# toonsegers/verifiable_mpc

Hardware: AMD Instinct MI355X
Metric: Ed25519 MSM scalar-mults/sec (higher is better)
Workload: dtype u32 (255-bit modular integers as 10 limbs of 25.5 bits, 32x32->64 multiply-adds)

## Files before the change

verifiable_mpc_amd/csrc/api.hip:

```cpp
#include <stdlib.h>

#include "common.h"


thread_local char vmpc_err_buf[512] = {0};

__attribute__((constructor)) static void vmpc_hw_queues_default() { setenv("GPU_MAX_HW_QUEUES", "16", 0); }

int vmpc_fr_check_dev(vmpc_ctx *ctx, const void *v, size_t n);

extern "C" const char *vmpc_last_error(void) { return vmpc_err_buf; }

const char *vmpc_getenv_experimental(const char *name) {
    const char *on = getenv("VMPC_EXPERIMENTAL");
    return (on && atoi(on) != 0) ? getenv(name) : nullptr;
}

extern "C" int vmpc_backend_info(char *buf, size_t buflen) {
    int n = 0;
    hipError_t e = hipGetDeviceCount(&n);
    if (e != hipSuccess || n <= 0) {
        if (buf && buflen) snprintf(buf, buflen, "no HIP device (%s)", hipGetErrorString(e));
        return VMPC_E_NODEV;
    }
    if (buf && buflen) {
        hipDeviceProp_t p;
        if (hipGetDeviceProperties(&p, 0) == hipSuccess)
            snprintf(buf, buflen, "%s %s cus=%d lds=%zu hbm=%.0fGiB devices=%d", p.gcnArchName, p.name,
                     p.multiProcessorCount, (size_t)p.sharedMemPerBlock,
                     (double)p.totalGlobalMem / (1024.0 * 1024.0 * 1024.0), n);
        else
            snprintf(buf, buflen, "devices=%d", n);
    }
    return n;
}

extern "C" int vmpc_ctx_create(int device, vmpc_ctx **out) {
    if (!out) return VMPC_E_INVAL;
    int n = 0;
    if (hipGetDeviceCount(&n) != hipSuccess || n <= 0) {
        snprintf(vmpc_err_buf, sizeof vmpc_err_buf, "no HIP device visible");
        return VMPC_E_NODEV;
    }
    if (device < 0 || device >= n) return VMPC_E_INVAL;
    VMPC_HIP_CHECK(hipSetDevice(device));
    vmpc_ctx *c = new vmpc_ctx();
    c->device = device;
    hipDeviceProp_t p;
    if (hipGetDeviceProperties(&p, device) == hipSuccess) {
        c->cu_count = p.multiProcessorCount;
        c->lds_optin = p.sharedMemPerBlockOptin ? p.sharedMemPerBlockOptin : p.sharedMemPerBlock;
    }
    hipError_t e = hipStreamCreateWithFlags(&c->stream, hipStreamNonBlocking);
    if (e != hipSuccess) {
        delete c;
        snprintf(vmpc_err_buf, sizeof vmpc_err_buf, "hipStreamCreate: %s", hipGetErrorString(e));
        return VMPC_E_HIP;
    }
    c->own_stream = true;
    e = hipMalloc((void **)&c->d_status, (VMPC_ST_WORDS + 16) * sizeof(uint32_t));
    if (e == hipSuccess) e = hipMemset(c->d_status, 0, (VMPC_ST_WORDS + 16) * sizeof(uint32_t));
    if (e != hipSuccess) {
        VMPC_IGNORE(hipStreamDestroy(c->stream));
        delete c;
        snprintf(vmpc_err_buf, sizeof vmpc_err_buf, "hipMalloc(status): %s", hipGetErrorString(e));
        return VMPC_E_HIP;
    }
    const char *w = getenv("VMPC_MSM_WINDOW");
    if (w) c->window_override = atoi(w);
    const char *fj = getenv("VMPC_FOLD_JUMP_DIGITS");
    if (fj && atoi(fj) == 4) c->fold_jump_digit_bits = 4;
    const char *sp = getenv("VMPC_SHORT_PATH");
    if (sp) c->short_path = atoi(sp) != 0;
    const char *bw = vmpc_getenv_experimental("VMPC_BUCKET_WGS_PER_CU");
    if (bw && atoi(bw) >= 0) c->bucket_wgs_per_cu = atoi(bw);
    const char *sf = vmpc_getenv_experimental("VMPC_SORT_FINE_BITS");
    if (sf && atoi(sf) >= 0) c->sort_fine_bits = atoi(sf);
    const char *rc = vmpc_getenv_experimental("VMPC_REDUCE_MAX_CHUNKS");
    if (rc && atoi(rc) >= 256 && atoi(rc) <= 32768) c->reduce_max_chunks = atoi(rc);
    const char *ro = vmpc_getenv_experimental("VMPC_REDUCE_CHUNKS");
    if (ro && atoi(ro) >= 64 && atoi(ro) <= 32768 && (atoi(ro) & (atoi(ro) - 1)) == 0) c->reduce_chunks_override = atoi(ro);
    const char *rt = vmpc_getenv_experimental("VMPC_REDUCE_TREE");
    if (rt) c->reduce_tree = atoi(rt) != 0;
    const char *ss = vmpc_getenv_experimental("VMPC_SEG_SHIFT_MIN");
    if (ss && atoi(ss) <= 0 && atoi(ss) >= -5) c->seg_shift_min = atoi(ss);
    *out = c;
    return VMPC_OK;
}

extern "C" int vmpc_ctx_destroy(vmpc_ctx *ctx) {
    if (!ctx) return VMPC_E_INVAL;
    if (ctx->p4_pool_busy) {
        snprintf(vmpc_err_buf, sizeof vmpc_err_buf, "vmpc_ctx_destroy: a vmpc_p4 of this context is still alive");
        return VMPC_E_INVAL;
    }
    VMPC_IGNORE(hipSetDevice(ctx->device));
    VMPC_IGNORE(hipStreamSynchronize(ctx->stream));
    for (auto &s : ctx->stages)
        for (auto &pr : s.pending) {
            VMPC_IGNORE(hipEventDestroy(pr.first));
            VMPC_IGNORE(hipEventDestroy(pr.second));
        }
    for (auto e : ctx->event_pool) VMPC_IGNORE(hipEventDestroy(e));
    if (ctx->xevent) VMPC_IGNORE(hipEventDestroy(ctx->xevent));
    if (ctx->ev_sorted) VMPC_IGNORE(hipEventDestroy(ctx->ev_sorted));
    if (ctx->ev_bucketed) VMPC_IGNORE(hipEventDestroy(ctx->ev_bucketed));
    if (ctx->pin_event) VMPC_IGNORE(hipEventDestroy(ctx->pin_event));
    if (ctx->pin) VMPC_IGNORE(hipHostFree(ctx->pin));
    if (ctx->ws) VMPC_IGNORE(hipFree(ctx->ws));
    if (ctx->p4_pool) VMPC_IGNORE(hipFree(ctx->p4_pool));
    if (ctx->p4_kblock) VMPC_IGNORE(hipFree(ctx->p4_kblock));
    if (ctx->d_status) VMPC_IGNORE(hipFree(ctx->d_status));
    if (ctx->short_cursors) VMPC_IGNORE(hipFree(ctx->short_cursors));
    if (ctx->ntt_twiddles) VMPC_IGNORE(hipFree(ctx->ntt_twiddles));
    if (ctx->own_stream) VMPC_IGNORE(hipStreamDestroy(ctx->stream));
    delete ctx;
    return VMPC_OK;
}

extern "C" int vmpc_ctx_set_stream(vmpc_ctx *ctx, void *hip_stream) {
    if (!ctx) return VMPC_E_INVAL;
    VMPC_HIP_CHECK(hipSetDevice(ctx->device));
    VMPC_HIP_CHECK(hipStreamSynchronize(ctx->stream));
    if (ctx->own_stream) {
        VMPC_IGNORE(hipStreamDestroy(ctx->stream));
        ctx->own_stream = false;
    }
    if (hip_stream) {
        ctx->stream = (hipStream_t)hip_stream;
    } else {
        VMPC_HIP_CHECK(hipStreamCreateWithFlags(&ctx->stream, hipStreamNonBlocking));
        ctx->own_stream = true;
    }
    return VMPC_OK;
}

extern "C" int vmpc_ctx_sync(vmpc_ctx *ctx) {
    if (!ctx) return VMPC_E_INVAL;
    VMPC_HIP_CHECK(hipSetDevice(ctx->device));
    VMPC_CHECK(vmpc_pinned_reserve(ctx, 0));
    volatile uint32_t *st = (volatile uint32_t *)((char *)ctx->pin_out + 2048);
    VMPC_HIP_CHECK(hipMemcpyAsync((void *)st, ctx->d_status, VMPC_ST_WORDS * sizeof(uint32_t), hipMemcpyDeviceToHost,
                                  ctx->stream));
    VMPC_HIP_CHECK(hipStreamSynchronize(ctx->stream));
    if (st[VMPC_ST_NONCANON]) {
        snprintf(vmpc_err_buf, sizeof vmpc_err_buf, "%u non-canonical scalar(s) (>= l) seen on device",
                 (unsigned)st[VMPC_ST_NONCANON]);
        VMPC_HIP_CHECK(hipMemsetAsync(ctx->d_status, 0, VMPC_ST_WORDS * sizeof(uint32_t), ctx->stream));
        VMPC_HIP_CHECK(hipStreamSynchronize(ctx->stream));
        return VMPC_E_NONCANON;
    }
    if (st[VMPC_ST_SHORT_OVERFLOW]) {
        snprintf(vmpc_err_buf, sizeof vmpc_err_buf,
                 "the short-commitment path met scalars beyond its fixed capacities: repeat the call on the general path "
                 "(vmpc_ctx_set_short_path(ctx, 0))");
        VMPC_HIP_CHECK(hipMemsetAsync(ctx->d_status, 0, VMPC_ST_WORDS * sizeof(uint32_t), ctx->stream));
        VMPC_HIP_CHECK(hipStreamSynchronize(ctx->stream));
        ctx->short_backoff = 64;
        return VMPC_E_AGAIN;
    }
    return VMPC_OK;
}

extern "C" int vmpc_ctx_debug_hold_wait(vmpc_ctx *ctx, int on) {
    if (!ctx) return VMPC_E_INVAL;
    ctx->stream_waits = on != 0;
    return VMPC_OK;
}

#define VMPC_DEBUG_DELAY_MAX_US 20000u
#define VMPC_DEBUG_DELAY_POLLS_PER_US 4u
__global__ __launch_bounds__(64) void k_debug_delay(uint32_t ticks, uint32_t max_polls) {
    if (threadIdx.x != 0) return;
    const uint64_t t0 = __builtin_amdgcn_s_memrealtime();
    for (uint32_t i = 0; i < max_polls; i++) {
        if (__builtin_amdgcn_s_memrealtime() - t0 >= (uint64_t)ticks) break;
        __builtin_amdgcn_s_sleep(16);
    }
}

extern "C" int vmpc_stream_debug_delay(void *hip_stream, int device, unsigned microseconds) {
    if (!hip_stream) return VMPC_E_INVAL;
    if (microseconds > VMPC_DEBUG_DELAY_MAX_US) {
        snprintf(vmpc_err_buf, sizeof vmpc_err_buf, "debug delay of %u us: the cap is %u us", microseconds,
                 VMPC_DEBUG_DELAY_MAX_US);
        return VMPC_E_RANGE;
    }
    if (microseconds == 0) return VMPC_OK;
    VMPC_HIP_CHECK(hipSetDevice(device));
    k_debug_delay<<<1, 64, 0, (hipStream_t)hip_stream>>>(microseconds * 100u,
                                                          microseconds * VMPC_DEBUG_DELAY_POLLS_PER_US + 64u);
    VMPC_KERNEL_CHECK();
    return VMPC_OK;
}

extern "C" int vmpc_ctx_debug_delay(vmpc_ctx *ctx, unsigned microseconds) {
    if (!ctx) return VMPC_E_INVAL;
    if (microseconds == 0 || microseconds > VMPC_DEBUG_DELAY_MAX_US)
        return vmpc_stream_debug_delay((void *)ctx->stream, ctx->device, microseconds);
    vmpc_stage_scope s(ctx, "debug_delay");
    return vmpc_stream_debug_delay((void *)ctx->stream, ctx->device, microseconds);
}

extern "C" int vmpc_ctx_set_short_path(vmpc_ctx *ctx, int on) {
    if (!ctx) return VMPC_E_INVAL;
    ctx->short_path = on ? 1 : 0;
    if (on == 2) ctx->short_backoff = 0;
    return VMPC_OK;
}

extern "C" int vmpc_ctx_get_short_path(vmpc_ctx *ctx, int *on) {
    if (!ctx || !on) return VMPC_E_INVAL;
    *on = ctx->short_path;
    return VMPC_OK;
}

extern "C" int vmpc_ctx_query(vmpc_ctx *ctx, int *done) {
    if (!ctx || !done) return VMPC_E_INVAL;
    VMPC_HIP_CHECK(hipSetDevice(ctx->device));
    hipError_t e = hipStreamQuery(ctx->stream);
    if (e == hipSuccess) {
        *done = 1;
    } else if (e == hipErrorNotReady) {
        (void)hipGetLastError();
        *done = 0;
    } else {
        VMPC_HIP_CHECK(e);
    }
    return VMPC_OK;
}

extern "C" int vmpc_ctx_wait_for(vmpc_ctx *waiter, vmpc_ctx *other) {
    if (!waiter || !other) return VMPC_E_INVAL;
    if (waiter == other || waiter->stream == other->stream) return VMPC_OK;
    VMPC_HIP_CHECK(hipSetDevice(other->device));
    if (!other->xevent) VMPC_HIP_CHECK(hipEventCreateWithFlags(&other->xevent, hipEventDisableTiming));
// ... 347 lines not shown
```

verifiable_mpc_amd/csrc/common.h:

```cpp
#pragma once
#include <hip/hip_runtime.h>
#include <stdint.h>
#include <stdio.h>
#include <string.h>

#include <string>
#include <vector>

#include "../../include/vmpc.h"

extern thread_local char vmpc_err_buf[512];

#define VMPC_HIP_CHECK(expr)                                                                  \
    do {                                                                                      \
        hipError_t _e = (expr);                                                               \
        if (_e != hipSuccess) {                                                               \
            snprintf(vmpc_err_buf, sizeof vmpc_err_buf, "%s:%d: %s -> %s", __FILE__, __LINE__, \
                     #expr, hipGetErrorString(_e));                                           \
            return VMPC_E_HIP;                                                                \
        }                                                                                     \
    } while (0)

#define VMPC_CHECK(expr)              \
    do {                              \
        int _r = (expr);              \
        if (_r != VMPC_OK) return _r; \
    } while (0)

#define VMPC_ST_NONCANON 0
#define VMPC_ST_SHORT_OVERFLOW 1
#define VMPC_ST_WORDS 4

struct vmpc_stage {
    const char *name;
    double ms = 0;
    uint64_t launches = 0;
    std::vector<std::pair<hipEvent_t, hipEvent_t>> pending;
};

struct vmpc_ctx {
    int device = 0;
    hipStream_t stream = nullptr;
    bool own_stream = false;
    void *ws = nullptr;
    size_t ws_bytes = 0;
    size_t ws_used = 0;
    uint32_t *d_status = nullptr;
    int window_override = 0;
    int bucket_wgs_per_cu = 0;
    int reduce_max_chunks = 32768;
    int reduce_chunks_override = 0;
    int short_path = 1;
    int short_backoff = 0;
    size_t lds_optin = 0;
    int fold_jump_digit_bits = 8;
    bool sort_wide_ready = false;
    bool short_ready = false;
    uint32_t *short_cursors = nullptr;
    int reduce_tree = 1;
    bool reduce_tree_ready = false;
    int seg_shift_min = -3;
    int sort_fine_bits = -1;
    int plan_fill_shift = 0;
    int cu_count = 256;
    vmpc_sort_view sort_view = {};
    bool sort_view_valid = false;
    hipEvent_t xevent = nullptr;
    hipStream_t bucket_stream = nullptr;
    hipEvent_t ev_sorted = nullptr, ev_bucketed = nullptr;
    hipStream_t stage_stream = nullptr;
    void *pin = nullptr;
    size_t pin_bytes = 0;
    hipEvent_t pin_event = nullptr;
    bool stream_waits = false;
    uint32_t *done_flag_dev = nullptr;
    uint32_t done_seq = 0;
    uint32_t p4_seq = 0;
    void *pin_out = nullptr;
    void *pin_out_dev = nullptr;
    void *p4_pool = nullptr;
    size_t p4_pool_bytes = 0;
    bool p4_pool_busy = false;
    void *p4_kblock = nullptr;
    int p4_kblock_rows = 0;
    uint8_t p4_kblock_key[64] = {0};
    int poly_product = 0;
    void *ntt_twiddles = nullptr;
    size_t ntt_arena_cap = 0;
    bool profile = false;
    std::vector<vmpc_stage> stages;
    std::vector<hipEvent_t> event_pool;
};

int vmpc_ws_reserve(vmpc_ctx *ctx, size_t total_bytes);
inline void *vmpc_ws_take(vmpc_ctx *ctx, size_t bytes) {
    size_t off = (ctx->ws_used + 255) & ~(size_t)255;
    ctx->ws_used = off + bytes;
    return (char *)ctx->ws + off;
}
int vmpc_stage_h2d(vmpc_ctx *ctx, void *dst, const void *src, size_t bytes);
int vmpc_pinned_reserve(vmpc_ctx *ctx, size_t bytes);
inline size_t vmpc_align(size_t b) { return (b + 255) & ~(size_t)255; }

int vmpc_ntt_poly_mul(vmpc_ctx *ctx, const void *a, size_t a_stride, size_t na, const void *b, size_t b_stride,
                      size_t nb, size_t k_lo, size_t k_cnt, void *out, size_t out_stride, size_t n_wit);

int vmpc_stage_begin(vmpc_ctx *ctx, const char *name);
void vmpc_stage_end(vmpc_ctx *ctx, int handle);

struct vmpc_stage_scope {
    vmpc_ctx *ctx;
    int h;
    vmpc_stage_scope(vmpc_ctx *c, const char *name) : ctx(c), h(vmpc_stage_begin(c, name)) {}
    ~vmpc_stage_scope() { vmpc_stage_end(ctx, h); }
};

const char *vmpc_getenv_experimental(const char *name);

#define VMPC_IGNORE(expr) ((void)(expr))
#define VMPC_KERNEL_CHECK() VMPC_HIP_CHECK(hipGetLastError())

#ifdef __HIPCC__
__device__ __forceinline__ void vmpc_publish_done(uint32_t *counter, uint32_t *flag, uint32_t seq) {
    __threadfence_system();
    if (atomicAdd(counter, 1u) == gridDim.x - 1) {
        *counter = 0;
        __threadfence_system();
        *(volatile uint32_t *)flag = seq;
    }
}
#endif
```

verifiable_mpc_amd/csrc/msm_reduce_tree.hip:

```cpp
#include "common.h"
#include "msm_sort.h"
#include "ge25519.h"
#include "ptio.h"
#include "quad.h"

#include "rt_tree.h"

template <bool HAS_U, bool LANE_P1>
__global__ void __launch_bounds__(LANE_P1 ? RT_THREADS / 2 : RT_THREADS)
k_msm_reduce_tree(const uint32_t *__restrict__ buckets, const uint32_t *__restrict__ counts, int nb, int G, int L,
                  uint32_t *__restrict__ out3) {
    extern __shared__ __align__(16) uint32_t rt_lds[];
    uint32_t *TA = rt_lds;
    uint32_t *RR = TA + RT_LEAVES * EXT_WORDS;
    uint32_t *DD = RR + (RT_LEAVES / 2) * EXT_WORDS;
    uint32_t *US = DD + (RT_LEAVES / 2) * EXT_WORDS;
    const int w = blockIdx.y, g = blockIdx.x;
    if (LANE_P1) {
        if (threadIdx.x < RT_LEAVES) {
            const int t = threadIdx.x;
            const int lo = (RT_LEAVES * g + t) * L;
            const uint32_t *bw = buckets + EXT_WORDS * ((size_t)w * nb + lo);
            const uint32_t *cw = counts + (size_t)w * (nb + 1) + lo + 1;
            ge_ext acc = ge_ext_identity(), sum = ge_ext_identity();
            bool have = false;
            for (int j = L - 1; j >= 0; j--) {
                if (cw[j]) {
                    const ge_ext B = ext_ld(bw + EXT_WORDS * j);
                    acc = have ? ge_add(acc, B) : B;
                    have = true;
                }
                if (j == L - 1) sum = acc;
                else if (have) sum = ge_add(sum, acc);
            }
            ext_st(TA + EXT_WORDS * t, acc);
            if (HAS_U) ext_st(US + EXT_WORDS * t, sum);
        }
    } else {
        const int t = threadIdx.x >> 2, q = threadIdx.x & 3;
        const int lo = (RT_LEAVES * g + t) * L;
        const uint32_t *bw = buckets + EXT_WORDS * ((size_t)w * nb + lo);
        const uint32_t *cw = counts + (size_t)w * (nb + 1) + lo + 1;
        fe acc = rt_identity(q), sum = acc;
        bool have = false;
        for (int j = L - 1; j >= 0; j--) {
            if (cw[j]) {
                const fe B = fe_ld(bw + EXT_WORDS * j + FE_LIMBS * q);
                acc = have ? rt_add(acc, B, q) : B;
                have = true;
            }
            if (HAS_U) {
                if (j == L - 1) sum = acc;
                else if (have) sum = rt_add(sum, acc, q);
            }
        }
        rt_st(TA, t, q, acc);
        if (HAS_U) rt_st(US, t, q, sum);
    }
    __syncthreads();
    rt_tree<!HAS_U, HAS_U, false>(TA, US, nullptr, RR, DD, RT_LEAVES);
    uint32_t *o = out3 + (size_t)EXT_WORDS * 3 * ((size_t)w * G + g);
    if (threadIdx.x < EXT_WORDS) {
        o[threadIdx.x] = HAS_U ? US[threadIdx.x] : TA[threadIdx.x];
        o[EXT_WORDS + threadIdx.x] = RR[threadIdx.x];
        o[2 * EXT_WORDS + threadIdx.x] = DD[threadIdx.x];
    }
}

__global__ void __launch_bounds__(RT_THREADS)
k_msm_reduce_combine(const uint32_t *__restrict__ in3, int G, int log2L, uint32_t *__restrict__ out,
                     uint32_t *__restrict__ out_packed, uint32_t *done_counter, uint32_t *done_flag, uint32_t done_seq,
                     int spl, uint32_t *__restrict__ reset, int reset_words, const uint32_t *__restrict__ poison,
                     int sub) {
    extern __shared__ __align__(16) uint32_t rt_lds[];
    uint32_t *TA = rt_lds;
    uint32_t *US = TA + (size_t)G * EXT_WORDS;
    uint32_t *EX = US + (size_t)G * EXT_WORDS;
    uint32_t *RR = EX + (size_t)G * EXT_WORDS;
    uint32_t *DD = RR + (size_t)(G > 1 ? G / 2 : 1) * EXT_WORDS;
    const int w = blockIdx.x;
    const uint32_t *src = in3 + (size_t)EXT_WORDS * 3 * (size_t)w * G * spl;
    if (reset)
        for (int i = threadIdx.x; i < reset_words; i += blockDim.x) reset[(size_t)w * reset_words + i] = 0;
    for (int i = threadIdx.x; i < G * 3 * EXT_WORDS; i += blockDim.x) {
        const int g = i / (3 * EXT_WORDS), r = i % (3 * EXT_WORDS), k = r / EXT_WORDS, e = r % EXT_WORDS;
        uint32_t *dst = k == 0 ? US : k == 1 ? EX : TA;
        dst[g * EXT_WORDS + e] = src[(size_t)g * spl * 3 * EXT_WORDS + r];
    }
    __syncthreads();
    for (int part = 1; part < spl; part++) {
        const int q = threadIdx.x & 3;
        for (int job = threadIdx.x >> 2; job < 3 * G; job += blockDim.x >> 2) {
            const int g = job / 3, k = job % 3;
            uint32_t *dst = k == 0 ? US : k == 1 ? EX : TA;
            const fe y = fe_ld(src + ((size_t)(g * spl + part) * 3 + k) * EXT_WORDS + FE_LIMBS * q);
            rt_st(dst, g, q, rt_add(rt_ld(dst, g, q), y, q));
        }
        __syncthreads();
    }
    if (G > 1) rt_tree<false, true, true>(TA, US, EX, RR, DD, G);
    if (threadIdx.x >= 64) return;
    const int q = threadIdx.x & 3;
    fe R = rt_ld(EX, 0, q);
    if (G > 1) R = rt_add(R, rt_ld(RR, 0, q), q);
    if (sub > 1 && G > 1) {
        const fe D = rt_ld(DD, 0, q);
        for (int h = w % sub; h > 0; h--) R = rt_add(R, D, q);
    }
    for (int k = 0; k < log2L; k++) R = quadD_dbl(R, q);
    R = rt_add(R, rt_ld(US, 0, q), q);
    if (poison && poison[w]) R = fe_zero();
    if (threadIdx.x < 4) {
        if (out_packed) fe_st8(out_packed + 32 * (size_t)w + 8 * q, R);
        else fe_st(out + EXT_WORDS * (size_t)w + FE_LIMBS * q, R);
    }
    __builtin_amdgcn_wave_barrier();
    if (out_packed && done_flag && threadIdx.x == 0) vmpc_publish_done(done_counter, done_flag, done_seq);
}

bool msm_reduce_tree_fits(const msm_plan &p) {
    if (p.chunks % RT_LEAVES != 0 || p.chunks * p.chunk_len != p.nb) return false;
    const int G = p.chunks / RT_LEAVES;
    return G >= 1 && (G <= 128 || (p.wide && G == 256)) && (G & (G - 1)) == 0 && p.chunk_len <= (p.wide ? 32 : 8) &&
           (p.chunk_len & (p.chunk_len - 1)) == 0;
}

int msm_reduce_tree_split(const msm_plan &p) {
    const int G = p.chunks / RT_LEAVES;
    return G > 128 ? G / 128 : 1;
}

int msm_reduce_tree(vmpc_ctx *ctx, const msm_plan &p, msm_ws &w, hipStream_t st, void *out_packed) {
    const int G = p.chunks / RT_LEAVES, L = p.chunk_len;
    const size_t lds_a1 = (size_t)(RT_LEAVES * 2) * EXT_WORDS * 4, lds_aU = (size_t)(RT_LEAVES * 3) * EXT_WORDS * 4;
    if (!ctx->reduce_tree_ready) {
        VMPC_HIP_CHECK(hipFuncSetAttribute((const void *)k_msm_reduce_tree<false, false>,
                                           hipFuncAttributeMaxDynamicSharedMemorySize, (int)lds_a1));
        VMPC_HIP_CHECK(hipFuncSetAttribute((const void *)k_msm_reduce_tree<true, false>,
                                           hipFuncAttributeMaxDynamicSharedMemorySize, (int)lds_aU));
        VMPC_HIP_CHECK(hipFuncSetAttribute((const void *)k_msm_reduce_tree<true, true>,
                                           hipFuncAttributeMaxDynamicSharedMemorySize, (int)lds_aU));
        VMPC_HIP_CHECK(hipFuncSetAttribute((const void *)k_msm_reduce_combine,
                                           hipFuncAttributeMaxDynamicSharedMemorySize, (int)((4 * 128 + 1) * EXT_WORDS * 4)));
        ctx->reduce_tree_ready = true;
    }
    const int sub = msm_reduce_tree_split(p);
    uint32_t *triples = w.partials + (size_t)EXT_WORDS * p.W * sub;
    if (L > 2)
        k_msm_reduce_tree<true, true><<<dim3(G, p.W), RT_THREADS / 2, lds_aU, st>>>(w.buckets, w.counts, p.nb, G, L, triples);
    else if (L > 1)
        k_msm_reduce_tree<true, false><<<dim3(G, p.W), RT_THREADS, lds_aU, st>>>(w.buckets, w.counts, p.nb, G, L, triples);
    else
        k_msm_reduce_tree<false, false><<<dim3(G, p.W), RT_THREADS, lds_a1, st>>>(w.buckets, w.counts, p.nb, G, L, triples);
    VMPC_KERNEL_CHECK();
    if (sub > 1 && out_packed) return VMPC_E_INVAL;
    k_msm_reduce_combine<<<p.W * sub, RT_THREADS, (size_t)(4 * (G / sub) + 1) * EXT_WORDS * 4, st>>>(
        triples, G / sub, msm_ilog2(L), w.partials, (uint32_t *)out_packed, ctx->d_status + VMPC_ST_WORDS,
        out_packed ? ctx->done_flag_dev : nullptr, ctx->done_seq, 1, nullptr, 0, nullptr, sub);
    if (out_packed) ctx->done_flag_dev = nullptr;
    VMPC_KERNEL_CHECK();
    return VMPC_OK;
}

int msm_reduce_combine_launch(vmpc_ctx *ctx, const uint32_t *triples, int W, int G, int spl, uint32_t *scratch_out,
                              void *out_packed, uint32_t *reset, int reset_words, const uint32_t *poison) {
    hipStream_t st = ctx->stream;
    if (!ctx->reduce_tree_ready && !ctx->short_ready)
        VMPC_HIP_CHECK(hipFuncSetAttribute((const void *)k_msm_reduce_combine,
                                           hipFuncAttributeMaxDynamicSharedMemorySize, (int)((4 * 128 + 1) * EXT_WORDS * 4)));
    const size_t lds_b = (size_t)(4 * G + 1) * EXT_WORDS * 4;
    k_msm_reduce_combine<<<W, RT_THREADS, lds_b, st>>>(triples, G, 0, scratch_out, (uint32_t *)out_packed,
                                                       ctx->d_status + VMPC_ST_WORDS, out_packed ? ctx->done_flag_dev : nullptr,
                                                       ctx->done_seq, spl, reset, reset_words, poison, 1);
    if (out_packed) ctx->done_flag_dev = nullptr;
    VMPC_KERNEL_CHECK();
    return VMPC_OK;
}
```

verifiable_mpc_amd/csrc/msm_sort.h:

```cpp
#pragma once
#include "common.h"

#define MSM_MAX_C 16
#define MSM_WIDE_C 20
#define MSM_WIDE_ROWS 13
#define MSM_BLOCK 256
#define MSM_SORT_BLOCK 1024
#define MSM_SEG 64
#define MSM_SEG_LOG2 6
#define MSM_FINISH_SERIAL 32
#ifndef MSM_REDUCE_CHUNKS
#define MSM_REDUCE_CHUNKS 4096
#endif

struct msm_plan {
    size_t n_main, n_extra, n_total;
    int scalar_bits;
    int c, W, nb, nb1;
    int seg_shift;
    int balanced;
    int LB;
    int NC;
    int J;
    int idx_bits;
    int fine_in_entry;
    int period;
    int top_row;
    uint32_t top_max_b;
    int LB_top;
    size_t n_pad;
    int chunks;
    int chunk_len;
    int red_blocks;
    int wide = 0;
    int chunks_per_row = 0;
    int col_bits = 0;
    size_t row_stride = 0;
    int fine_cap = 12288;
};
inline size_t msm_seg_len(const msm_plan &p) { return (size_t)1 << (MSM_SEG_LOG2 + p.seg_shift); }


typedef uint4 msm_task;
#define MSM_TASK_SPLIT 1u

struct msm_ws {
    uint32_t *entries;
    uint32_t *hist1;
    size_t hist1_n;
    uint32_t *stage1;
    uint32_t *counts, *starts, *sorted;
    uint32_t *buckets;
    uint32_t *partials;
    uint32_t *nseg, *seg_starts, *block_hist, *block_base, *heavy_list, *ctrl;
    uint32_t *seg_partial;
    msm_task *tasks;
    int16_t *digits;
    void *scan_ws;
    size_t total;
    uint32_t plan_blocks;
    size_t t_max;
};

struct msm_modulus {
    uint32_t v[8];
};

void msm_make_plan(vmpc_ctx *ctx, size_t n_main, size_t n_extra, int scalar_bits, msm_plan &p,
                   const msm_modulus *modulus = nullptr);
void msm_plan_geometry(vmpc_ctx *ctx, msm_plan &p);
void msm_layout(const msm_plan &p, msm_ws &w, char *base, size_t entry_bytes, size_t acc_bytes);
bool msm_reduce_tree_fits(const msm_plan &p);
int msm_reduce_tree_split(const msm_plan &p);
int msm_reduce_tree(vmpc_ctx *ctx, const msm_plan &p, msm_ws &w, hipStream_t st, void *out_packed);
int msm_sort_stage(vmpc_ctx *ctx, const msm_plan &p, msm_ws &w, const void *scalars, size_t n,
                   const void *extra_scalars, const msm_modulus &modulus);
int msm_sort_digits(vmpc_ctx *ctx, const msm_plan &p, msm_ws &w);
int msm_recode_wide_batch(vmpc_ctx *ctx, const void *const *scalars, size_t n_main, const void *const *extra_scalars,
                          int K, size_t extra_pos, size_t n_extra, size_t row_stride, int32_t *digits32,
                          size_t digits_per_commitment, const msm_modulus &modulus);
int msm_recode_rows(vmpc_ctx *ctx, const void *scalars, size_t n_main, const void *extra_scalars,
                    size_t extra_pos, size_t n_extra, size_t n_pad, int16_t *digits, int c, int W, int rows,
                    const msm_modulus &modulus);
int msm_recode_rows_batch(vmpc_ctx *ctx, const void *const *scalars, size_t n_main, const void *const *extra_scalars,
                          int K, size_t extra_pos, size_t n_extra, size_t n_pad, int16_t *digits,
                          size_t digits_per_commitment, int c, int W, int rows, const msm_modulus &modulus);

static inline int msm_ilog2(int v) {
    int r = 0;
    while ((1 << r) < v) r++;
    return r;
}

__host__ __device__ __forceinline__ uint32_t msm_seg_count(uint32_t cnt, uint32_t seg_log) {
    return (cnt + (1u << seg_log) - 1u) >> seg_log;
}
__device__ __forceinline__ void msm_seg_range(uint32_t cnt, uint32_t ns, uint32_t sidx, uint32_t seg, int balanced,
                                              uint32_t &off, uint32_t &len) {
    if (ns <= 1) {
        off = 0;
        len = cnt;
        return;
    }
    if (!balanced) {
        off = sidx * seg;
        len = cnt - off < seg ? cnt - off : seg;
        return;
    }
    const uint32_t q = cnt / ns, r = cnt - q * ns;
    off = sidx * q + (sidx < r ? sidx : r);
    len = q + (sidx < r ? 1u : 0u);
}

__device__ __forceinline__ size_t msm_bucket_slot(uint32_t ci, int nb1) {
    uint32_t w = ci / (uint32_t)nb1;
    return (size_t)ci - w - 1;
}

__device__ __forceinline__ msm_task msm_make_task(uint32_t ci, uint32_t start, uint32_t cnt, uint32_t ns, uint32_t sidx,
                                                  uint32_t seg, int balanced, uint32_t seg_start, int nb1) {
    uint32_t off, len;
    msm_seg_range(cnt, ns, sidx, seg, balanced, off, len);
    if (ns <= 1) return make_uint4(start + off, len, (uint32_t)msm_bucket_slot(ci, nb1), 0u);
    return make_uint4(start + off, len, seg_start + sidx, MSM_TASK_SPLIT);
}
```

verifiable_mpc_amd/csrc/msm_sort.hip:

```cpp
#include "common.h"
#include "msm_sort.h"
#include "scan.h"

#define SORT_T 8192
#define SORT_BLOCK 1024
#define SORT_WAVES (SORT_BLOCK / 64)
#define SORT_FINE_CAP 12288

__device__ __forceinline__ uint32_t msm_seg_class(uint32_t rem, int seg_shift) {
    return seg_shift > 0 ? (rem + (1u << seg_shift) - 1u) >> seg_shift : rem;
}

__device__ __forceinline__ void load_u32x8(uint32_t dst[8], const uint32_t *src) {
    const uint4 *p = reinterpret_cast<const uint4 *>(src);
    uint4 a = p[0], b = p[1];
    dst[0] = a.x; dst[1] = a.y; dst[2] = a.z; dst[3] = a.w;
    dst[4] = b.x; dst[5] = b.y; dst[6] = b.z; dst[7] = b.w;
}

struct msm_recode_batch {
    const uint32_t *sc[16];
    const uint32_t *sc_extra[16];
};

// ... 546 lines not shown
    __shared__ uint32_t scratch[16];
    for (int w = 0; w < W; w++) {
        msm_ranks_window(block_hist, NC, W, w, ctrl, part);
        __syncthreads();
    }
    msm_classes_body(ctrl, W, class_base, scratch);
}

__global__ void __launch_bounds__(512)
k_msm_plan2(const uint32_t *__restrict__ counts, const uint32_t *__restrict__ starts,
            const uint32_t *__restrict__ seg_starts, int NC, int W, int NF, int top_row, int period, int NF_top, int nb1,
            int seg_shift, int balanced,
            const uint32_t *__restrict__ class_base, const uint32_t *__restrict__ block_rank,
            msm_task *__restrict__ tasks) {
    const uint32_t seg_log = (uint32_t)(MSM_SEG_LOG2 + seg_shift);
    __shared__ uint32_t cur[MSM_SEG + 1], first[MSM_SEG + 1];
    const uint32_t block = blockIdx.x;
    const int w = block / NC, cb = block % NC;
    if (threadIdx.x >= 1 && threadIdx.x <= MSM_SEG) {
        cur[threadIdx.x] = 0;
        first[threadIdx.x] = class_base[(MSM_SEG - threadIdx.x) * W + w] +
                             block_rank[(size_t)block * MSM_SEG + (threadIdx.x - 1)];
    }
    __syncthreads();
    if (w % period == top_row) NF = NF_top;
    if (threadIdx.x >= (unsigned)NF) return;
    const size_t ci = (size_t)w * nb1 + 1 + (size_t)cb * NF + threadIdx.x;
    const uint32_t cnt = counts[ci];
    const uint32_t ns = msm_seg_count(cnt, seg_log);
    if (ns == 0) return;
    const uint32_t start = starts[ci], seg = 1u << seg_log;
    const uint32_t seg_start = ns > 1 ? seg_starts[ci] : 0u;
    if (balanced) {
        const uint32_t bin = msm_seg_class((cnt + ns - 1u) / ns, seg_shift);
        const uint32_t base = first[bin] + atomicAdd(&cur[bin], ns);
        for (uint32_t sidx = 0; sidx < ns; sidx++)
            tasks[base + sidx] = msm_make_task((uint32_t)ci, start, cnt, ns, sidx, seg, 1, seg_start, nb1);
        return;
    }
    const uint32_t full = cnt >> seg_log, rem = cnt & (seg - 1u);
    if (rem) {
        const uint32_t bin = msm_seg_class(rem, seg_shift);
        tasks[first[bin] + atomicAdd(&cur[bin], 1u)] =
            msm_make_task((uint32_t)ci, start, cnt, ns, full, seg, 0, seg_start, nb1);
    }
    if (full) {
        const uint32_t base = first[MSM_SEG] + atomicAdd(&cur[MSM_SEG], full);
        for (uint32_t sidx = 0; sidx < full; sidx++)
            tasks[base + sidx] = msm_make_task((uint32_t)ci, start, cnt, ns, sidx, seg, 0, seg_start, nb1);
    }
}

static int msm_pick_window(size_t n, int scalar_bits) {
    if (scalar_bits == 253) return n > (1u << 13) ? 16 : 11;
    double best = 1e300;
    int best_c = 4;
    for (int c = 4; c <= MSM_MAX_C; c++) {
        int W = (scalar_bits + 2 + c - 1) / c;
        double cost = (double)W * ((double)n + 2.5 * (double)(1u << (c - 1)));
        if (cost < best) {
            best = cost;
            best_c = c;
        }
    }
    return best_c;
}

static uint32_t msm_top_max_bucket(const msm_modulus &mod, int c, int W) {
    uint32_t m1[8];
    uint64_t borrow = 1;
    for (int i = 0; i < 8; i++) {
        uint64_t v = (uint64_t)mod.v[i] - borrow;
        m1[i] = (uint32_t)v;
        borrow = (v >> 63) & 1;
    }
    const int shift = c * (W - 1);
    if (shift >= 256) return 0;
    uint64_t top = 0;
    for (int bit = 0; bit < 32 && shift + bit < 256; bit++)
        top |= (uint64_t)((m1[(shift + bit) >> 5] >> ((shift + bit) & 31)) & 1u) << bit;
    for (int bit = shift + 32; bit < 256; bit++)
        if ((m1[bit >> 5] >> (bit & 31)) & 1u) return 0xffffffffu;
    return (uint32_t)(top > 0xfffffffeull ? 0xffffffffull : top);
}

void msm_make_plan(vmpc_ctx *ctx, size_t n_main, size_t n_extra, int scalar_bits, msm_plan &p,
                   const msm_modulus *modulus) {
    p.n_main = n_main;
    p.n_extra = n_extra;
    p.n_total = n_main + n_extra;
    p.scalar_bits = scalar_bits;
    p.c = ctx->window_override ? ctx->window_override : msm_pick_window(p.n_total, scalar_bits);
    if (p.c < 4) p.c = 4;
    if (p.c > MSM_MAX_C) p.c = MSM_MAX_C;
    p.W = (scalar_bits + 2 + p.c - 1) / p.c;
    while (p.W > 64) {
        p.c++;
        p.W = (scalar_bits + 2 + p.c - 1) / p.c;
    }
    p.top_row = -1;
    p.top_max_b = 0;
    p.period = p.W;
    if (modulus) {
        p.top_row = p.W - 1;
        p.top_max_b = msm_top_max_bucket(*modulus, p.c, p.W);
    }
    msm_plan_geometry(ctx, p);
}

void msm_plan_geometry(vmpc_ctx *ctx, msm_plan &p) {
    if (p.period <= 0 || p.period > p.W) p.period = p.W;
    p.nb = 1 << (p.c - 1);
    p.nb1 = p.nb + 1;
    p.n_pad = (p.n_total + 7) & ~(size_t)7;
    p.idx_bits = 1;
    while (((size_t)1 << p.idx_bits) < p.n_pad) p.idx_bits++;
    const int nc_target = p.n_total >= ((size_t)1 << 22) ? 256 : 512;
    int lb = p.c - 1;
    if (lb > 9) lb = 9;
    while (lb > 0 && (p.nb >> lb) < nc_target && (p.n_total >> (p.c - 1 - lb)) > 8192) lb--;
    if (ctx->sort_fine_bits >= 0 && ctx->sort_fine_bits <= 9 && ctx->sort_fine_bits <= p.c - 1 &&
        (p.nb >> ctx->sort_fine_bits) <= 4096)
        lb = ctx->sort_fine_bits;
    p.fine_cap = SORT_FINE_CAP;
    if (p.wide) {
        lb = 9;
        while (lb > 6 && (p.n_total >> (p.c - 1 - lb)) > 14336) lb--;
        p.idx_bits = p.col_bits;
        p.fine_cap = 16384;
    }
    p.LB = lb;
    p.NC = p.nb >> lb;
    p.fine_in_entry = p.idx_bits + lb <= 31;
    p.LB_top = lb;
    if (p.top_row >= 0) {
        int lt = 0;
        while (lt < lb && (p.top_max_b >> lt) > (uint32_t)(p.NC - 1)) lt++;
        p.LB_top = lt;
    }
    p.J = (int)((p.n_pad + SORT_T - 1) / SORT_T);
    p.balanced = p.scalar_bits == 253 ? 1 : 0;
    const size_t work = ((size_t)p.W * p.n_total) >> ctx->plan_fill_shift;
    p.seg_shift = 0;
    while (p.seg_shift < 4 && (((size_t)MSM_SEG << p.seg_shift) << 18) < work) p.seg_shift++;
    while (p.seg_shift > ctx->seg_shift_min && (((size_t)MSM_SEG >> -(p.seg_shift - 1)) << 18) >= work)
        p.seg_shift--;
    int chunks = MSM_REDUCE_CHUNKS;
    while (chunks * 2 * p.W <= MSM_REDUCE_CHUNKS * 16 &&
           chunks * 2 <= (p.wide && ctx->reduce_max_chunks == 32768 ? 65536 : ctx->reduce_max_chunks))
        chunks *= 2;
    while (chunks * p.W > MSM_REDUCE_CHUNKS * 16 && chunks > 256) chunks /= 2;
    if (ctx->reduce_chunks_override >= 64) chunks = ctx->reduce_chunks_override;
    if (chunks > p.nb) chunks = p.nb;
    p.chunks = chunks;
    p.chunk_len = p.nb / chunks;
    p.red_blocks = (chunks + MSM_BLOCK - 1) / MSM_BLOCK;
}

void msm_layout(const msm_plan &p, msm_ws &w, char *base, size_t entry_bytes, size_t acc_bytes) {
    size_t off = 0;
    auto take = [&](size_t bytes) {
        size_t o = off;
        off += vmpc_align(bytes);
        return base ? (void *)(base + o) : (void *)nullptr;
    };
    size_t nbk = (size_t)p.W * p.nb1;
    w.entries = (uint32_t *)take(p.n_total * entry_bytes);
    w.digits = (int16_t *)take((size_t)p.W * p.n_pad * (p.wide ? 4 : 2));
    w.hist1_n = (size_t)p.W * p.NC * p.J;
    w.hist1 = (uint32_t *)take((w.hist1_n + 1) * 4);
    w.counts = (uint32_t *)take(nbk * 4);
    w.starts = (uint32_t *)take(nbk * 4);
    w.stage1 = (uint32_t *)take((size_t)p.W * p.n_total * 4);
    w.sorted = (uint32_t *)take((size_t)p.W * p.n_total * 4);
    w.buckets = (uint32_t *)take((size_t)p.W * p.nb * acc_bytes);
    w.partials = (uint32_t *)take((size_t)p.W * (3 * p.red_blocks + 4) * acc_bytes);
    size_t m_max = (size_t)p.W * p.n_total;
    size_t nonempty_max = m_max < (size_t)p.W * p.nb ? m_max : (size_t)p.W * p.nb;
    w.t_max = m_max / msm_seg_len(p) + nonempty_max;
    w.plan_blocks = (uint32_t)(p.W * p.NC);
    size_t hist_n = (size_t)MSM_SEG * w.plan_blocks;
    w.block_hist = (uint32_t *)take(hist_n * 4);
    w.block_base = (uint32_t *)take((size_t)MSM_SEG * p.W * 4);
    w.nseg = (uint32_t *)take(nbk * 4);
    w.seg_starts = (uint32_t *)take(nbk * 4);
    w.heavy_list = (uint32_t *)take(nbk * 4);
    w.ctrl = (uint32_t *)take((16 + (size_t)MSM_SEG * p.W) * 4);
    w.tasks = (msm_task *)take(w.t_max * sizeof(msm_task));
    w.seg_partial = (uint32_t *)take(w.t_max * acc_bytes);
    size_t scan_n = hist_n;
    if (w.hist1_n > scan_n) scan_n = w.hist1_n;
    w.scan_ws = take(vmpc_scan_ws_bytes(scan_n, 4));
    w.total = off;
}

int msm_sort_stage(vmpc_ctx *ctx, const msm_plan &p, msm_ws &w, const void *scalars, size_t n,
                   const void *extra_scalars, const msm_modulus &modulus) {
    hipStream_t st = ctx->stream;
    const size_t n_total = p.n_total;
    const unsigned gb = (unsigned)((p.n_pad + MSM_BLOCK - 1) / MSM_BLOCK);
    {
        vmpc_stage_scope s(ctx, "msm_recode");
        k_msm_recode<<<gb, MSM_BLOCK, 0, st>>>((const uint32_t *)scalars, n,
                                              (const uint32_t *)extra_scalars, n, n_total - n, p.n_pad, w.digits, p.c,
                                              p.W, p.W, p.n_pad, modulus, ctx->d_status);
        VMPC_KERNEL_CHECK();
    }
    return msm_sort_digits(ctx, p, w);
}

int msm_recode_rows(vmpc_ctx *ctx, const void *scalars, size_t n_main, const void *extra_scalars,
                    size_t extra_pos, size_t n_extra, size_t n_pad, int16_t *digits, int c, int W, int rows,
                    const msm_modulus &modulus) {
    vmpc_stage_scope s(ctx, "msm_recode");
    const int wpr = W / rows;
    k_msm_recode<<<(unsigned)((n_pad + MSM_BLOCK - 1) / MSM_BLOCK), MSM_BLOCK, 0, ctx->stream>>>(
        (const uint32_t *)scalars, n_main, (const uint32_t *)extra_scalars, extra_pos, n_extra, n_pad, digits, c,
        W, wpr, (size_t)rows * n_pad, modulus, ctx->d_status);
    VMPC_KERNEL_CHECK();
    return VMPC_OK;
}

int msm_recode_rows_batch(vmpc_ctx *ctx, const void *const *scalars, size_t n_main, const void *const *extra_scalars,
                          int K, size_t extra_pos, size_t n_extra, size_t n_pad, int16_t *digits,
                          size_t digits_per_commitment, int c, int W, int rows, const msm_modulus &modulus) {
    vmpc_stage_scope s(ctx, "msm_recode");
    msm_recode_batch b;
    memset(&b, 0, sizeof b);
    for (int k = 0; k < K; k++) {
        b.sc[k] = (const uint32_t *)scalars[k];
        b.sc_extra[k] = extra_scalars ? (const uint32_t *)extra_scalars[k] : nullptr;
    }
    const int wpr = W / rows;
    k_msm_recode_batch<<<dim3((unsigned)((n_pad + MSM_BLOCK - 1) / MSM_BLOCK), K), MSM_BLOCK, 0, ctx->stream>>>(
        b, n_main, extra_pos, n_extra, n_pad, digits, digits_per_commitment, c, W, wpr, (size_t)rows * n_pad, modulus,
        ctx->d_status);
    VMPC_KERNEL_CHECK();
    return VMPC_OK;
}

int msm_recode_wide_batch(vmpc_ctx *ctx, const void *const *scalars, size_t n_main, const void *const *extra_scalars,
                          int K, size_t extra_pos, size_t n_extra, size_t row_stride, int32_t *digits32,
                          size_t digits_per_commitment, const msm_modulus &modulus) {
    vmpc_stage_scope s(ctx, "msm_recode");
    msm_recode_batch b;
    memset(&b, 0, sizeof b);
    for (int k = 0; k < K; k++) {
        b.sc[k] = (const uint32_t *)scalars[k];
        b.sc_extra[k] = extra_scalars ? (const uint32_t *)extra_scalars[k] : nullptr;
    }
    k_msm_recode_wide<<<dim3((unsigned)((row_stride + MSM_BLOCK - 1) / MSM_BLOCK), K), MSM_BLOCK, 0, ctx->stream>>>(
        b, n_main, extra_pos, n_extra, row_stride, digits32, digits_per_commitment, modulus, ctx->d_status);
    VMPC_KERNEL_CHECK();
    return VMPC_OK;
}

template <bool FINE_IN_ENTRY, int CAP>
static int msm_launch_fine(vmpc_ctx *ctx, const msm_plan &p, msm_ws &w) {
    hipStream_t st = ctx->stream;
    const unsigned grid = (unsigned)p.NC * (unsigned)p.W;
    const size_t dyn = CAP > SORT_FINE_CAP ? (size_t)CAP * 4 : 0;
    if (dyn && !ctx->sort_wide_ready) {
        VMPC_HIP_CHECK(hipFuncSetAttribute((const void *)k_sort_fine<FINE_IN_ENTRY, CAP>,
                                           hipFuncAttributeMaxDynamicSharedMemorySize, (int)dyn));
        VMPC_HIP_CHECK(hipFuncSetAttribute((const void *)k_sort_fine_big<FINE_IN_ENTRY, CAP>,
                                           hipFuncAttributeMaxDynamicSharedMemorySize, (int)dyn));
        ctx->sort_wide_ready = true;
    }
    k_sort_fine<FINE_IN_ENTRY, CAP><<<grid, SORT_BLOCK, dyn, st>>>(
        w.stage1, w.hist1, p.NC, p.W, p.LB, p.top_row, p.period, p.LB_top, p.J, p.idx_bits, p.chunks_per_row,
        (uint32_t)p.row_stride, p.nb1, w.digits, p.n_pad, w.counts, w.starts, w.sorted, p.seg_shift, p.balanced, w.nseg,
        w.block_hist, w.heavy_list, w.seg_starts, w.ctrl);
    k_sort_fine_big<FINE_IN_ENTRY, CAP><<<grid, SORT_BLOCK, dyn, st>>>(
        w.stage1, w.hist1, p.NC, p.W, p.LB, p.top_row, p.period, p.LB_top, p.J, p.idx_bits, p.chunks_per_row,
        (uint32_t)p.row_stride, p.nb1, w.digits, p.n_pad, w.starts, w.sorted, w.ctrl);
    VMPC_KERNEL_CHECK();
    return VMPC_OK;
}

int msm_sort_digits(vmpc_ctx *ctx, const msm_plan &p, msm_ws &w) {
    hipStream_t st = ctx->stream;
    if (p.wide && (!p.fine_in_entry || p.chunks_per_row <= 0 || p.J != p.chunks_per_row * MSM_WIDE_ROWS ||
                   p.n_pad != (size_t)p.J * SORT_T || p.row_stride != (size_t)p.chunks_per_row * SORT_T))
        return VMPC_E_INVAL;
    static const int xcd = getenv("VMPC_WIDE_XCD") ? atoi(getenv("VMPC_WIDE_XCD")) : 1;
    const dim3 chunk_grid(p.wide ? 8 * ((p.J + 7) / 8) : p.J, p.W);
    {
        vmpc_stage_scope s(ctx, "msm_hist");
        if (p.wide)
            k_sort_hist1<true><<<chunk_grid, SORT_BLOCK, (size_t)p.NC * 4, st>>>(w.digits, p.n_pad, p.NC, p.LB, p.top_row,
                                                                                p.period, p.LB_top, p.J, xcd, w.hist1, w.ctrl);
        else
            k_sort_hist1<false><<<chunk_grid, SORT_BLOCK, (size_t)p.NC * 4, st>>>(w.digits, p.n_pad, p.NC, p.LB, p.top_row,
                                                                                 p.period, p.LB_top, p.J, 0, w.hist1, w.ctrl);
        VMPC_KERNEL_CHECK();
        VMPC_CHECK((vmpc_exclusive_scan<uint32_t, uint32_t>(st, w.hist1, w.hist1, w.hist1_n, w.scan_ws,
                                                            w.hist1 + w.hist1_n)));
    }
    {
        vmpc_stage_scope s(ctx, "msm_part");
        const size_t lds_bytes = ((size_t)3 * p.NC + 16 + (p.wide ? 2 : 1) * SORT_T) * 4;
        if (p.wide) {
            if (lds_bytes > 48 * 1024)
                VMPC_HIP_CHECK(hipFuncSetAttribute((const void *)k_sort_part1<true>,
                                                   hipFuncAttributeMaxDynamicSharedMemorySize, (int)lds_bytes));
            k_sort_part1<true><<<chunk_grid, SORT_BLOCK, lds_bytes, st>>>(
// ... 49 lines not shown
```

verifiable_mpc_amd/csrc/rt_tree.h:

```cpp
#pragma once
#include "common.h"
#include "ge25519.h"
#include "ptio.h"
#include "quad.h"

#define RT_THREADS 1024
#define RT_LEAVES 256

__device__ __forceinline__ fe rt_ld(const uint32_t *arr, int idx, int q) { return fe_ld(arr + EXT_WORDS * (size_t)idx + FE_LIMBS * q); }
__device__ __forceinline__ void rt_st(uint32_t *arr, int idx, int q, const fe &v) { fe_st(arr + EXT_WORDS * (size_t)idx + FE_LIMBS * q, v); }
__device__ __forceinline__ fe rt_identity(int q) { return (q == 1 || q == 2) ? fe_one() : fe_zero(); }
__device__ __forceinline__ fe rt_add(const fe &P, const fe &Q, int q) { return quadD_add_cached(P, quadD_to_cached(Q, q), q); }
__device__ __forceinline__ int rt_pad16(int v) { return (v + 15) & ~15; }

template <bool KEEP_T, bool HAS_U, bool HAS_E>
__device__ __forceinline__ void rt_tree(uint32_t *TA, uint32_t *US, uint32_t *EX, uint32_t *RR, uint32_t *DD, int n) {
    enum { OP_ADD = 0, OP_R = 1, OP_D = 2, OP_PAIR = 3 };
    const int qd = threadIdx.x >> 2, q = threadIdx.x & 3, nquads = blockDim.x >> 2;
    int lvl = 0;
    for (int m = n >> 1; m >= 1; m >>= 1, lvl++) {
        const int nplain = (lvl == 0 ? 0 : (KEEP_T ? 1 : 0)) + (HAS_U ? 1 : 0) + (HAS_E ? 1 : 0);
        int cnt = m;
        while (rt_pad16(cnt * nplain) + (lvl == 0 ? 1 : 2) * rt_pad16(cnt) > nquads) cnt >>= 1;
        const int nA = rt_pad16(cnt * nplain), nC = rt_pad16(cnt);
        const int total = nA + (lvl == 0 ? 1 : 2) * nC;
        int op, jl;
        bool on;
        uint32_t *arr;
        {
            int plain_at = lvl == 0 ? nC : 0;
            if (qd >= plain_at && qd < plain_at + nA) {
                int pk = (qd - plain_at) / cnt;
                jl = (qd - plain_at) % cnt;
                on = pk < nplain;
                op = OP_ADD;
                arr = US;
                if (KEEP_T && lvl > 0) {
                    if (pk == 0) arr = TA;
                    pk--;
                }
                if (HAS_U) {
                    if (pk == 0) arr = US;
                    pk--;
                }
                if (HAS_E && pk == 0) arr = EX;
            } else if (lvl == 0) {
                op = OP_PAIR; jl = qd; on = qd < cnt; arr = TA;
            } else if (qd < nA + nC) {
                op = OP_R; jl = qd - nA; on = jl < cnt; arr = RR;
            } else {
                op = OP_D; jl = qd - nA - nC; on = jl < cnt; arr = DD;
            }
            if (!on) arr = TA;
        }
        const bool wave_on = (qd & ~15) < total;
        for (int j0 = 0; j0 < m; j0 += cnt) {
            const int j = j0 + jl, jj = on ? j : 0;
            fe x, y, z;
            if (wave_on) {
                x = rt_ld(arr, 2 * jj, q);
                y = rt_ld(arr, 2 * jj + 1, q);
                if (op == OP_R) z = rt_ld(DD, 2 * jj + 1, q);
            }
            __syncthreads();
            if (wave_on) {
                const fe s = rt_add(x, y, q);
                fe s2 = s;
                if (op == OP_R) s2 = rt_add(s, z, q);
                else if (op == OP_D || op == OP_PAIR) s2 = quadD_dbl(s, q);
                if (on) {
                    if (op == OP_PAIR) {
                        if (KEEP_T) rt_st(TA, j, q, s);
                        rt_st(RR, j, q, y);
                        rt_st(DD, j, q, s2);
                    } else {
                        rt_st(arr, j, q, s2);
                    }
                }
            }
            __syncthreads();
        }
    }
}
```

Measured before the change: 1.447 billion.

## Add split wide-window bucket reduction with per-chunk sums, tree, and combine

```diff
diff --git a/verifiable_mpc_amd/csrc/api.hip b/verifiable_mpc_amd/csrc/api.hip
--- a/verifiable_mpc_amd/csrc/api.hip
+++ b/verifiable_mpc_amd/csrc/api.hip
@@ -82,6 +82,10 @@
     if (ro && atoi(ro) >= 64 && atoi(ro) <= 32768 && (atoi(ro) & (atoi(ro) - 1)) == 0) c->reduce_chunks_override = atoi(ro);
     const char *rt = vmpc_getenv_experimental("VMPC_REDUCE_TREE");
     if (rt) c->reduce_tree = atoi(rt) != 0;
+    const char *wr = vmpc_getenv_experimental("VMPC_WIDE_REDUCE");
+    if (wr) c->wide_reduce = atoi(wr) != 0;
+    const char *wl = vmpc_getenv_experimental("VMPC_WIDE_REDUCE_LEN");
+    if (wl && atoi(wl) >= 8 && atoi(wl) <= 64 && (atoi(wl) & (atoi(wl) - 1)) == 0) c->wide_reduce_len = atoi(wl);
     const char *ss = vmpc_getenv_experimental("VMPC_SEG_SHIFT_MIN");
     if (ss && atoi(ss) <= 0 && atoi(ss) >= -5) c->seg_shift_min = atoi(ss);
     *out = c;
diff --git a/verifiable_mpc_amd/csrc/common.h b/verifiable_mpc_amd/csrc/common.h
--- a/verifiable_mpc_amd/csrc/common.h
+++ b/verifiable_mpc_amd/csrc/common.h
@@ -59,6 +59,9 @@
     uint32_t *short_cursors = nullptr;
     int reduce_tree = 1;
     bool reduce_tree_ready = false;
+    int wide_reduce = -1;
+    int wide_reduce_len = 32;
+    bool reduce_wide_ready = false;
     int seg_shift_min = -3;
     int sort_fine_bits = -1;
     int plan_fill_shift = 0;
diff --git a/verifiable_mpc_amd/csrc/msm_reduce_tree.hip b/verifiable_mpc_amd/csrc/msm_reduce_tree.hip
--- a/verifiable_mpc_amd/csrc/msm_reduce_tree.hip
+++ b/verifiable_mpc_amd/csrc/msm_reduce_tree.hip
@@ -118,19 +118,124 @@
     if (out_packed && done_flag && threadIdx.x == 0) vmpc_publish_done(done_counter, done_flag, done_seq);
 }
 
+#define RT_WIDE_THREADS 256
+__global__ void __launch_bounds__(MSM_BLOCK, 3)
+k_msm_chunk_sums(uint32_t *__restrict__ buckets, const uint32_t *__restrict__ counts, int nb, int L) {
+    const int w = blockIdx.y;
+    const size_t lo = ((size_t)blockIdx.x * MSM_BLOCK + threadIdx.x) * L;
+    uint32_t *bw = buckets + EXT_WORDS * ((size_t)w * nb + lo);
+    const uint32_t *cw = counts + (size_t)w * (nb + 1) + lo + 1;
+    ge_ext acc = ge_ext_identity(), sum = ge_ext_identity();
+    bool have = false;
+    for (int j = L - 1; j >= 0; j--) {
+        if (cw[j]) {
+            const ge_ext B = ext_ld(bw + EXT_WORDS * j);
+            acc = have ? ge_add(acc, B) : B;
+            have = true;
+        }
+        if (j == L - 1) sum = acc;
+        else if (have) sum = ge_add(sum, acc);
+    }
+    ext_st(bw, acc);
+    ext_st(bw + EXT_WORDS, sum);
+}
+
+__global__ void __launch_bounds__(RT_WIDE_THREADS, 4)
+k_msm_wide_tree(const uint32_t *__restrict__ buckets, int nb, int G, int L, uint32_t *__restrict__ out3) {
+    __builtin_amdgcn_s_setprio(3);
+    extern __shared__ __align__(16) uint32_t rt_lds[];
+    uint32_t *RR = rt_lds;
+    uint32_t *DD = RR + (RT_LEAVES / 2) * EXT_WORDS;
+    uint32_t *US = DD + (RT_LEAVES / 2) * EXT_WORDS;
+    const int w = blockIdx.y, g = blockIdx.x;
+    const int qd = threadIdx.x >> 2, q = threadIdx.x & 3, nquads = blockDim.x >> 2;
+    const uint32_t *leaf = buckets + EXT_WORDS * ((size_t)w * nb + (size_t)RT_LEAVES * g * L);
+    const size_t stride = (size_t)L * EXT_WORDS;
+    for (int job = qd; job < RT_LEAVES; job += nquads) {
+        const bool weighted = job < RT_LEAVES / 2;
+        rt_level0_global(leaf + (weighted ? 0 : EXT_WORDS), stride, job & (RT_LEAVES / 2 - 1), q, weighted, US, RR, DD);
+    }
+    __syncthreads();
+    rt_tree<false, true, false>(RR, US, nullptr, RR, DD, RT_LEAVES, 1);
+    uint32_t *o = out3 + (size_t)EXT_WORDS * 3 * ((size_t)w * G + g);
+    if (threadIdx.x < EXT_WORDS) {
+        o[threadIdx.x] = US[threadIdx.x];
+        o[EXT_WORDS + threadIdx.x] = RR[threadIdx.x];
+        o[2 * EXT_WORDS + threadIdx.x] = DD[threadIdx.x];
+    }
+}
+
+__global__ void __launch_bounds__(RT_WIDE_THREADS, 4)
+k_msm_wide_combine(const uint32_t *__restrict__ in3, int G, int log2L, uint32_t *__restrict__ out,
+                   uint32_t *__restrict__ out_packed, uint32_t *done_counter, uint32_t *done_flag, uint32_t done_seq) {
+    __builtin_amdgcn_s_setprio(3);
+    extern __shared__ __align__(16) uint32_t rt_lds[];
+    const int H = G / 2;
+    uint32_t *US = rt_lds;
+    uint32_t *EX = US + (size_t)H * EXT_WORDS;
+    uint32_t *RR = EX + (size_t)H * EXT_WORDS;
+    uint32_t *DD = RR + (size_t)H * EXT_WORDS;
+    const int w = blockIdx.x;
+    const int qd = threadIdx.x >> 2, q = threadIdx.x & 3, nquads = blockDim.x >> 2;
+    const uint32_t *src = in3 + (size_t)EXT_WORDS * 3 * (size_t)w * G;
+    for (int job = qd; job < 3 * H; job += nquads) {
+        const int k = job / H;
+        rt_level0_global(src + k * EXT_WORDS, 3 * EXT_WORDS, job % H, q, k == 2, k == 0 ? US : EX, RR, DD);
+    }
+    __syncthreads();
+    rt_tree<false, true, true>(RR, US, EX, RR, DD, G, 1);
+    if (threadIdx.x >= 64) return;
+    fe R = rt_add(rt_ld(EX, 0, q), rt_ld(RR, 0, q), q);
+    for (int k = 0; k < log2L; k++) R = quadD_dbl(R, q);
+    R = rt_add(R, rt_ld(US, 0, q), q);
+    if (threadIdx.x < 4) {
+        if (out_packed) fe_st8(out_packed + 32 * (size_t)w + 8 * q, R);
+        else fe_st(out + EXT_WORDS * (size_t)w + FE_LIMBS * q, R);
+    }
+    __builtin_amdgcn_wave_barrier();
+    if (out_packed && done_flag && threadIdx.x == 0) vmpc_publish_done(done_counter, done_flag, done_seq);
+}
+
+static int msm_reduce_wide(vmpc_ctx *ctx, const msm_plan &p, msm_ws &w, hipStream_t st, void *out_packed) {
+    const int G = p.chunks / RT_LEAVES, L = p.chunk_len;
+    const size_t lds_t = (size_t)(RT_LEAVES / 2 * 3) * EXT_WORDS * 4, lds_c = (size_t)(4 * (G / 2)) * EXT_WORDS * 4;
+    if (!ctx->reduce_wide_ready) {
+        VMPC_HIP_CHECK(hipFuncSetAttribute((const void *)k_msm_wide_tree, hipFuncAttributeMaxDynamicSharedMemorySize,
+                                           (int)lds_t));
+        VMPC_HIP_CHECK(hipFuncSetAttribute((const void *)k_msm_wide_combine, hipFuncAttributeMaxDynamicSharedMemorySize,
+                                           (int)((4 * 128) * EXT_WORDS * 4)));
+        ctx->reduce_wide_ready = true;
+    }
+    uint32_t *triples = w.partials + (size_t)EXT_WORDS * p.W;
+    k_msm_chunk_sums<<<dim3(p.chunks / MSM_BLOCK, p.W), MSM_BLOCK, 0, st>>>(w.buckets, w.counts, p.nb, L);
+    VMPC_KERNEL_CHECK();
+    k_msm_wide_tree<<<dim3(G, p.W), RT_WIDE_THREADS, lds_t, st>>>(w.buckets, p.nb, G, L, triples);
+    VMPC_KERNEL_CHECK();
+    k_msm_wide_combine<<<p.W, RT_WIDE_THREADS, lds_c, st>>>(triples, G, msm_ilog2(L), w.partials, (uint32_t *)out_packed,
+                                                          ctx->d_status + VMPC_ST_WORDS,
+                                                          out_packed ? ctx->done_flag_dev : nullptr, ctx->done_seq);
+    if (out_packed) ctx->done_flag_dev = nullptr;
+    VMPC_KERNEL_CHECK();
+    return VMPC_OK;
+}
+
 bool msm_reduce_tree_fits(const msm_plan &p) {
     if (p.chunks % RT_LEAVES != 0 || p.chunks * p.chunk_len != p.nb) return false;
     const int G = p.chunks / RT_LEAVES;
+    if (p.reduce_split)
+        return G >= 4 && G <= 256 && (G & (G - 1)) == 0 && p.chunk_len >= 2 && (p.chunk_len & (p.chunk_len - 1)) == 0;
     return G >= 1 && (G <= 128 || (p.wide && G == 256)) && (G & (G - 1)) == 0 && p.chunk_len <= (p.wide ? 32 : 8) &&
            (p.chunk_len & (p.chunk_len - 1)) == 0;
 }
 
 int msm_reduce_tree_split(const msm_plan &p) {
     const int G = p.chunks / RT_LEAVES;
+    if (p.reduce_split) return 1;
     return G > 128 ? G / 128 : 1;
 }
 
 int msm_reduce_tree(vmpc_ctx *ctx, const msm_plan &p, msm_ws &w, hipStream_t st, void *out_packed) {
+    if (p.reduce_split) return msm_reduce_wide(ctx, p, w, st, out_packed);
     const int G = p.chunks / RT_LEAVES, L = p.chunk_len;
     const size_t lds_a1 = (size_t)(RT_LEAVES * 2) * EXT_WORDS * 4, lds_aU = (size_t)(RT_LEAVES * 3) * EXT_WORDS * 4;
     if (!ctx->reduce_tree_ready) {
diff --git a/verifiable_mpc_amd/csrc/msm_sort.h b/verifiable_mpc_amd/csrc/msm_sort.h
--- a/verifiable_mpc_amd/csrc/msm_sort.h
+++ b/verifiable_mpc_amd/csrc/msm_sort.h
@@ -4,6 +4,7 @@
 #define MSM_MAX_C 16
 #define MSM_WIDE_C 20
 #define MSM_WIDE_ROWS 13
+#define MSM_WIDE_SPLIT_MIN_K 3
 #define MSM_BLOCK 256
 #define MSM_SORT_BLOCK 1024
 #define MSM_SEG 64
@@ -32,6 +33,7 @@
     int chunks;
     int chunk_len;
     int red_blocks;
+    int reduce_split = 0;
     int wide = 0;
     int chunks_per_row = 0;
     int col_bits = 0;
diff --git a/verifiable_mpc_amd/csrc/msm_sort.hip b/verifiable_mpc_amd/csrc/msm_sort.hip
--- a/verifiable_mpc_amd/csrc/msm_sort.hip
+++ b/verifiable_mpc_amd/csrc/msm_sort.hip
@@ -722,6 +722,12 @@
     while (chunks * p.W > MSM_REDUCE_CHUNKS * 16 && chunks > 256) chunks /= 2;
     if (ctx->reduce_chunks_override >= 64) chunks = ctx->reduce_chunks_override;
     if (chunks > p.nb) chunks = p.nb;
+    p.reduce_split = 0;
+    if (p.wide && ctx->reduce_tree && ctx->reduce_chunks_override < 64 &&
+        (ctx->wide_reduce < 0 ? p.W >= MSM_WIDE_SPLIT_MIN_K : ctx->wide_reduce != 0)) {
+        p.reduce_split = 1;
+        chunks = p.nb / ctx->wide_reduce_len;
+    }
     p.chunks = chunks;
     p.chunk_len = p.nb / chunks;
     p.red_blocks = (chunks + MSM_BLOCK - 1) / MSM_BLOCK;
diff --git a/verifiable_mpc_amd/csrc/rt_tree.h b/verifiable_mpc_amd/csrc/rt_tree.h
--- a/verifiable_mpc_amd/csrc/rt_tree.h
+++ b/verifiable_mpc_amd/csrc/rt_tree.h
@@ -13,12 +13,26 @@
 __device__ __forceinline__ fe rt_add(const fe &P, const fe &Q, int q) { return quadD_add_cached(P, quadD_to_cached(Q, q), q); }
 __device__ __forceinline__ int rt_pad16(int v) { return (v + 15) & ~15; }
 
+__device__ __forceinline__ void rt_level0_global(const uint32_t *src, size_t stride, int j, int q, bool weighted,
+                                                 uint32_t *PL, uint32_t *RR, uint32_t *DD) {
+    const fe x = fe_ld(src + (size_t)(2 * j) * stride + FE_LIMBS * q);
+    const fe y = fe_ld(src + (size_t)(2 * j + 1) * stride + FE_LIMBS * q);
+    const fe s = rt_add(x, y, q);
+    if (weighted) {
+        rt_st(RR, j, q, y);
+        rt_st(DD, j, q, quadD_dbl(s, q));
+    } else {
+        rt_st(PL, j, q, s);
+    }
+}
+
 template <bool KEEP_T, bool HAS_U, bool HAS_E>
-__device__ __forceinline__ void rt_tree(uint32_t *TA, uint32_t *US, uint32_t *EX, uint32_t *RR, uint32_t *DD, int n) {
+__device__ __forceinline__ void rt_tree(uint32_t *TA, uint32_t *US, uint32_t *EX, uint32_t *RR, uint32_t *DD, int n,
+                                        int lvl0 = 0) {
     enum { OP_ADD = 0, OP_R = 1, OP_D = 2, OP_PAIR = 3 };
     const int qd = threadIdx.x >> 2, q = threadIdx.x & 3, nquads = blockDim.x >> 2;
-    int lvl = 0;
-    for (int m = n >> 1; m >= 1; m >>= 1, lvl++) {
+    int lvl = lvl0;
+    for (int m = (n >> 1) >> lvl0; m >= 1; m >>= 1, lvl++) {
         const int nplain = (lvl == 0 ? 0 : (KEEP_T ? 1 : 0)) + (HAS_U ? 1 : 0) + (HAS_E ? 1 : 0);
         int cnt = m;
         while (rt_pad16(cnt * nplain) + (lvl == 0 ? 1 : 2) * rt_pad16(cnt) > nquads) cnt >>= 1;
```

New measurement: 1.450 billion, median of 6. No clear change (+0.2%).
